# zprodev/zlib.es

Hardware: AMD Instinct MI355X
Metric: GiB/s deflate+inflate round trip, 64 MiB buffers (uncompressed bytes / wall), bit-exact vs reference (higher is better)
Workload: dtype u8; 1 GPU; random64: 1 x 64 MiB xorshift buffer(s) per GPU (seed 12345+index), deflate then inflate, HBM-resident; bytes_per_buffer=67108864, compressed_bytes=67176156, parallelism=independent buffers, one per GPU

## Files before the change

### zlib.es_amd/csrc/zes_api.hip

```cpp
#include "../../include/zes.h"
#include "zes_kernels.h"
#include "zes_chain.h"

#include <algorithm>
#include <atomic>
#include <condition_variable>
#include <cstdio>
#include <cstddef>
#include <cstdlib>
#include <cstring>
#include <chrono>
#include <functional>
#include <future>
#include <initializer_list>
#include <deque>
#include <map>
#include <mutex>
#include <string>
#include <thread>
#include <vector>

extern "C" int zes_gen(uint8_t* out, uint64_t n, uint32_t kind, uint32_t seed);

namespace {
// ... 808 lines not shown
  if ((rc = ensure(g.hists, (size_t)nblk * 320 * 4))) return rc;
  if ((rc = ensure(g.codes, (size_t)nblk * 320 * 4))) return rc;
  if ((rc = ensure(g.hdrs, (size_t)nblk * ZES_HDR_WORDS * 4))) return rc;
  if ((rc = ensure(g.adler, (size_t)nbuf * 16))) return rc;
  if ((rc = ensure(g.res, sizeof(ZesRes) * nbuf))) return rc;
  ZesBuf* dbufs = (ZesBuf*)g.bufs.p;
  ZesBlk* dblks = (ZesBlk*)g.blks.p;
  unsigned long long* adler = (unsigned long long*)g.adler.p;
  if (nbuf > 1) {
    if (nbuf <= DEFLATE_TABLE_BUFS) {
      memcpy(g.pinned->def.table, hb.data(), sizeof(ZesBuf) * nbuf);
      HIPCHK(hipMemcpyAsync(g.bufs.p, g.pinned->def.table, sizeof(ZesBuf) * nbuf, hipMemcpyHostToDevice, g.stream));
    } else {
      HIPCHK(hipMemcpy(g.bufs.p, hb.data(), sizeof(ZesBuf) * nbuf, hipMemcpyHostToDevice));
    }
  }
  {
    Timed t("k_make_blks");
    const uint32_t nthr = std::max(nblk, 2u * nbuf);
    hipLaunchKernelGGL(k_make_blks, dim3((nthr + 255) / 256), dim3(256), 0, g.stream, hb[0], nbuf, dbufs, dblks, nblk, adler);
  }
  {
    HIPCHK(hipEventRecord(g.ev_a0, g.stream));
    HIPCHK(hipStreamWaitEvent(g.s_adler, g.ev_a0, 0));
    Timed t("k_adler", g.s_adler);
    if (nbuf == 1) {
      const uint32_t nch = (uint32_t)((hb[0].n + ADLER_CHUNK - 1) / ADLER_CHUNK);
      hipLaunchKernelGGL(k_adler, dim3(nch), dim3(ADLER_THREADS), 0, g.s_adler, d_in, hb[0].in_off, hb[0].n, adler);
    } else {
      hipLaunchKernelGGL(k_adler_blocks, dim3(nblk), dim3(ADLER_THREADS), 0, g.s_adler, d_in, dbufs, dblks, adler);
    }
  }
  HIPCHK(hipEventRecord(g.ev_a1, g.s_adler));
  const bool sort_dbg = getenv("ZES_DEBUG_PHASES") != nullptr;
  if (sort_dbg && (rc = phases_arm(zes_sort_set_dbg, nblk))) return rc;
  static const bool use_index = getenv("ZES_NO_INDEX") == nullptr;
  rc = launch_lz77(d_in, nblk, use_index, nbuf > 1 && nblk > 256, sort_dbg, [&]() -> int {
    if (!sort_dbg) return ZES_OK;
    return phases_print(zes_sort_set_dbg, nblk, 7,
                        "zes sort steps (avg cycles over %u blocks): zero %.0f count %.0f flag %.0f compact %.0f stage %.0f three passes %.0f sd/inv %.0f\n");
  });
  if (rc) return rc;
  if (sort_dbg) {
    if ((rc = phases_print(zes_parse_set_dbg, nblk, 7, "zes parse steps (avg cycles over %u blocks): A %.0f B %.0f C %.0f D1 %.0f D2 %.0f D3 %.0f out %.0f\n"))) return rc;
    if ((rc = phases_arm(zes_huff_set_dbg, nblk))) return rc;
  }
  ZesRes* res_direct = (nbuf <= DEFLATE_DIRECT_BUFS && g.pinned_dev) ? g.pinned_dev->def.res : nullptr;
  {
    Timed t("k_huff");
    hipLaunchKernelGGL(k_huff, dim3(nblk), dim3(HUFF_THREADS_HOST), 0, g.stream, dblks, (const uint32_t*)g.hists.p,
                       (uint32_t*)g.codes.p, (uint32_t*)g.hdrs.p);
  }
  if (sort_dbg && (rc = phases_print(zes_huff_set_dbg, nblk, 7,
                                     "zes huff steps (avg cycles over %u blocks): lit/len lengths %.0f distance lengths %.0f codes %.0f run-length coding %.0f its code %.0f header bits %.0f totals+out %.0f\n")))
    return rc;
  {
    HIPCHK(hipStreamWaitEvent(g.stream, g.ev_a1, 0));
    Timed t("k_layout");
    hipLaunchKernelGGL(k_layout, dim3(nbuf), dim3(256), 0, g.stream, d_out, dbufs, dblks, adler, res_direct ? res_direct : (ZesRes*)g.res.p);
  }
  {
    Timed t("k_emit");
    hipLaunchKernelGGL(k_emit, dim3(nblk), dim3(EMIT_THREADS), 0, g.stream, d_out, dbufs, dblks, (uint32_t*)g.idx_a.p,
                       (const uint32_t*)g.codes.p, (const uint32_t*)g.hdrs.p);
  }
  HIPCHK(hipGetLastError());
  ZesRes* r = g.pinned->def.res;
  if (nbuf > DEFLATE_DIRECT_BUFS) {
    if (nbuf > g.res_more_n) {
      if (g.res_more) HIPCHK(hipHostFree(g.res_more));
      g.res_more = nullptr;
      g.res_more_n = 0;
      HIPCHK(hipHostMalloc((void**)&g.res_more, sizeof(ZesRes) * nbuf * 2, hipHostMallocDefault));
      g.res_more_n = (size_t)nbuf * 2;
    }
    r = g.res_more;
  }
  if (!res_direct) HIPCHK(hipMemcpyAsync(r, g.res.p, sizeof(ZesRes) * nbuf, hipMemcpyDeviceToHost, g.stream));
  if (one && one->defer) return ZES_OK;
  HIPCHK(hipStreamSynchronize(g.stream));
  collect_times();
  for (uint32_t k = 0; k < nbuf; k++) {
    out_len[live[k]] = r[k].out_len;
    status[live[k]] = r[k].status;
  }
  if (one) one->adler = r[0].aux;
  return ZES_OK;
}

int deflate_one(const uint8_t* d_in, uint64_t in_off, uint64_t n, uint8_t* d_out, uint64_t out_off, uint64_t cap, uint64_t* out_len,
                DeflateRange* range = nullptr) {
  int32_t st = 0;
  const int rc = deflate_batch_core(d_in, &in_off, &n, d_out, &out_off, &cap, out_len, &st, 1, range);
  return rc ? rc : st;
}

int read_res(ZesRes* out) {
  HIPCHK(hipMemcpyAsync(&g.pinned->res1, g.res.p, sizeof(ZesRes), hipMemcpyDeviceToHost, g.stream));
  HIPCHK(hipStreamSynchronize(g.stream));
  *out = g.pinned->res1;
  return ZES_OK;
}

struct InfJob {
  uint64_t in_off, c, out_off, cap;
  uint64_t out_len;
  int status;
// ... 4809 lines not shown
```

### zlib.es_amd/csrc/zes_deflate.hip

```cpp
#include "zes_common.h"
#include "zes_kernels.h"

__device__ static inline uint32_t lds_ld32u(const uint8_t* s, uint32_t off) {
  const uint32_t* w = reinterpret_cast<const uint32_t*>(s);
  uint32_t i = off >> 2;
  uint32_t lo = w[i], hi = w[i + 1];
  return __builtin_amdgcn_alignbyte(hi, lo, off & 3u);
}

__device__ static inline void stage_block(uint8_t* s, const uint8_t* g, uint32_t bytes, uint32_t padded) {
  const uint32_t tid = threadIdx.x, nth = blockDim.x;
  const uint32_t mis = (uint32_t)((uintptr_t)g & 15u);
  if (mis == 0) {
    const uint4* g4 = reinterpret_cast<const uint4*>(g);
    uint4* s4 = reinterpret_cast<uint4*>(s);
    const uint32_t full = bytes >> 4;
    for (uint32_t i = tid; i < full; i += nth) s4[i] = g4[i];
    for (uint32_t i = (full << 4) + tid; i < padded; i += nth) s[i] = i < bytes ? g[i] : (uint8_t)0;
  } else {
    for (uint32_t i = tid; i < padded; i += nth) s[i] = i < bytes ? g[i] : (uint8_t)0;
  }
}

__device__ unsigned long long* g_sort_dbg = nullptr;
// ... 1783 lines not shown
      const uint32_t c = cb + k;
      const unsigned long long mk = mks[k];
      if ((mk >> lane) & 1ull) {
        const uint32_t m = ism[k] ? mw[k] : 0u;
        const uint32_t rank = (uint32_t)__popcll(mk & zes_lanemask_lt());
        uint32_t tv;
        if (m & ZES_TOK_MATCH) {
          tv = m;
          atomicAdd(&S.lh[257u + zes_len_code(zes_tok_len(m))], 1u);
          atomicAdd(&S.dh[zes_dist_code(zes_tok_dist(m))], 1u);
        } else {
          tv = by[k];
          atomicAdd(&S.lh[tv], 1u);
        }
        to[S.u.d.cpre[c] + rank] = tv;
      }
    }
  }
  __syncthreads();
  PSTAMP(6);
  if (tid == 0) {
    S.lh[256] = 1;
    blks[g].ntok = total;
  }
  __syncthreads();
  uint32_t* hg = hists + (uint64_t)g * 320;
  for (uint32_t i = tid; i < 288; i += PARSE_THREADS) hg[i] = S.lh[i];
  if (tid < 32) hg[288 + tid] = S.dh[tid];
  PSTAMP(7);
}

__global__ __launch_bounds__(PARSE_THREADS) void k_lz_parse(const uint8_t* __restrict__ d_in, const ZesBuf* __restrict__ bufs,
                                                            ZesBlk* __restrict__ blks, const uint32_t* __restrict__ match_in,
                                                            uint32_t* __restrict__ tok_out, uint32_t* __restrict__ hists,
                                                            const uint32_t* __restrict__ tmask_all, const uint32_t* __restrict__ mlist_all) {
  __shared__ __align__(16) ParseSmemT<false> S;
  parse_body<false>(S, d_in, bufs, blks, match_in, tok_out, hists, tmask_all, mlist_all);
}
__global__ __launch_bounds__(PARSE_THREADS, 8) void k_lz_parse_small(const uint8_t* __restrict__ d_in, const ZesBuf* __restrict__ bufs,
                                                                     ZesBlk* __restrict__ blks, const uint32_t* __restrict__ match_in,
                                                                     uint32_t* __restrict__ tok_out, uint32_t* __restrict__ hists,
                                                                     const uint32_t* __restrict__ tmask_all,
                                                                     const uint32_t* __restrict__ mlist_all) {
  __shared__ __align__(16) ParseSmemT<true> S;
  parse_body<true>(S, d_in, bufs, blks, match_in, tok_out, hists, tmask_all, mlist_all);
}

__device__ unsigned long long* g_huff_dbg = nullptr;
void zes_huff_set_dbg(unsigned long long* p) { (void)hipMemcpyToSymbol(HIP_SYMBOL(g_huff_dbg), &p, sizeof p); }
#define USTAMP(i)                                                                                        \
  do {                                                                                                   \
    if (g_huff_dbg && threadIdx.x == 0) g_huff_dbg[(size_t)blockIdx.x * 8 + (i)] = (unsigned long long)clock64(); \
  } while (0)
#define HUFF_THREADS 256
#define PM_MAXN 288
struct HuffSmem {
  uint32_t hist[320];
  uint32_t lw[PM_MAXN];
  uint16_t lsym[PM_MAXN];
  uint32_t w[2][2 * PM_MAXN];
  uint32_t pk[PM_MAXN];
  uint16_t leafpos[15][PM_MAXN];
  uint32_t a_k[16];
  uint8_t lens[320];
  uint8_t clens[32];
  uint16_t codes[320];
  uint16_t ccodes[32];
  uint8_t rl_sym[320];
  uint8_t rl_val[320];
  uint32_t nrl;
  uint32_t hdr[ZES_HDR_WORDS];
  uint32_t hdr_bits;
  uint32_t total_bits;
  uint32_t ccount[16], cfirst[16], crun[16];
  uint16_t cwave[HUFF_THREADS / 64][16];
  uint8_t cl[320];
  uint16_t run_tok[320];
  uint32_t wsum[HUFF_THREADS / 64];
  unsigned long long starts[5];
};

__device__ static inline uint32_t lower_bound_u32(const uint32_t* a, uint32_t n, uint32_t v) {
  uint32_t lo = 0, hi = n;
  while (lo < hi) {
    uint32_t mid = (lo + hi) >> 1;
    if (a[mid] < v) lo = mid + 1; else hi = mid;
  }
  return lo;
}
__device__ static inline uint32_t upper_bound_u32(const uint32_t* a, uint32_t n, uint32_t v) {
  uint32_t lo = 0, hi = n;
  while (lo < hi) {
    uint32_t mid = (lo + hi) >> 1;
    if (a[mid] <= v) lo = mid + 1; else hi = mid;
  }
  return lo;
}

__device__ static void pm_lengths(HuffSmem& S, const uint32_t* hist, uint32_t nsym, uint32_t L, uint8_t* lens) {
  const uint32_t tid = threadIdx.x, lane = tid & 63u;
  __syncthreads();
  uint32_t n = 0;
  for (uint32_t s0 = 0; s0 < nsym; s0 += HUFF_THREADS) n += (uint32_t)__syncthreads_count(s0 + tid < nsym && hist[s0 + tid] != 0u);
  for (uint32_t s = tid; s < nsym; s += HUFF_THREADS) {
    lens[s] = 0;
    const uint32_t c = hist[s];
    if (c) {
      uint32_t rank = 0;
      for (uint32_t j = 0; j < nsym; j++) {
        const uint32_t cj = hist[j];
        rank += (cj != 0) && (cj < c || (cj == c && j < s));
      }
      S.lw[rank] = c;
      S.lsym[rank] = (uint16_t)s;
    }
  }
  __syncthreads();
  if (n == 0) return;
  if (n == 1) {
    if (tid == 0) lens[S.lsym[0]] = 1;
    __syncthreads();
    return;
  }
  for (uint32_t i = tid; i < n; i += HUFF_THREADS) {
    S.w[0][i] = S.lw[i];
    S.leafpos[0][i] = (uint16_t)i;
  }
  uint32_t len_prev = n & ~1u;
  uint32_t sel = 0;
  __syncthreads();
  static_assert(PM_MAXN <= 2 * HUFF_THREADS && PM_MAXN < 512, "two items of either kind per thread, nine search steps");
  const uint32_t st0 = 1u << (31u - (uint32_t)__builtin_clz(n));
  const bool wide = n > HUFF_THREADS;
  for (uint32_t k = 1; k < L; k++) {
    const uint32_t np = len_prev >> 1;
    const uint2* wp2 = reinterpret_cast<const uint2*>(S.w[sel]);
    uint32_t* wc = S.w[sel ^ 1];
    const uint32_t i0 = min(tid, n - 1u), i1 = min(tid + HUFF_THREADS, n - 1u);
    const uint32_t j0 = min(tid, np - 1u), j1 = min(tid + HUFF_THREADS, np - 1u);
    const uint32_t lv0 = S.lw[i0], lv1 = S.lw[i1];
    const uint2 pa = wp2[j0], pb = wp2[j1];
    const uint32_t pv0 = pa.x + pa.y, pv1 = pb.x + pb.y;
    uint32_t ll0 = 0, ll1 = 0, pl0 = 0, pl1 = 0;
    if (!wide) {
#pragma unroll 1
      for (uint32_t st = st0; st; st >>= 1) {
        const uint32_t ml = ll0 + st, mp = pl0 + st;
        const uint2 x = wp2[min(ml, np) - 1u];
        const uint32_t y = S.lw[min(mp, n) - 1u];
        ll0 = (ml <= np && x.x + x.y < lv0) ? ml : ll0;
        pl0 = (mp <= n && y <= pv0) ? mp : pl0;
      }
    } else {
#pragma unroll 1
      for (uint32_t st = st0; st; st >>= 1) {
        const uint32_t ml0 = ll0 + st, ml1 = ll1 + st, mp0 = pl0 + st, mp1 = pl1 + st;
        const uint2 x0 = wp2[min(ml0, np) - 1u], x1 = wp2[min(ml1, np) - 1u];
        const uint32_t y0 = S.lw[min(mp0, n) - 1u], y1 = S.lw[min(mp1, n) - 1u];
        ll0 = (ml0 <= np && x0.x + x0.y < lv0) ? ml0 : ll0;
        ll1 = (ml1 <= np && x1.x + x1.y < lv1) ? ml1 : ll1;
        pl0 = (mp0 <= n && y0 <= pv0) ? mp0 : pl0;
        pl1 = (mp1 <= n && y1 <= pv1) ? mp1 : pl1;
      }
    }
    if (tid < n) {
      wc[tid + ll0] = lv0;
      S.leafpos[k][tid] = (uint16_t)(tid + ll0);
    }
    if (tid < np) wc[tid + pl0] = pv0;
    if (wide) {
      if (tid + HUFF_THREADS < n) {
        wc[tid + HUFF_THREADS + ll1] = lv1;
        S.leafpos[k][tid + HUFF_THREADS] = (uint16_t)(tid + HUFF_THREADS + ll1);
      }
      if (tid + HUFF_THREADS < np) wc[tid + HUFF_THREADS + pl1] = pv1;
    }
    len_prev = (n + np) & ~1u;
    sel ^= 1;
    __syncthreads();
  }
  if (tid < 64u) {
    uint32_t m = len_prev;
    for (int k = (int)L - 1; k >= 0; k--) {
      uint32_t a = 0;
#pragma unroll
      for (uint32_t c = 0; c < (PM_MAXN + 63) / 64; c++) {
        const uint32_t i = c * 64u + lane;
        a += (uint32_t)__popcll(__ballot(i < n && S.leafpos[k][min(i, n - 1u)] < m));
      }
      if (lane == 0) S.a_k[k] = a;
      m = 2u * (m - a);
    }
  }
  __syncthreads();
  for (uint32_t i = tid; i < n; i += HUFF_THREADS) {
    uint32_t l = 0;
    for (uint32_t k = 0; k < L; k++) l += (S.a_k[k] > i);
    lens[S.lsym[i]] = (uint8_t)l;
  }
  __syncthreads();
}

__device__ static void canon_codes(HuffSmem& S, const uint8_t* lens, uint32_t nsym, uint16_t* codes) {
  const uint32_t tid = threadIdx.x, lane = tid & 63u, wave = tid >> 6;
  if (tid < 16) {
    S.ccount[tid] = 0;
    S.crun[tid] = 0;
  }
  __syncthreads();
  for (uint32_t s = tid; s < nsym; s += HUFF_THREADS)
    if (lens[s]) atomicAdd(&S.ccount[lens[s]], 1u);
  __syncthreads();
  if (tid == 0) {
    uint32_t code = 0;
    for (uint32_t l = 1; l < 16; l++) {
      S.cfirst[l] = code;
      code = (code + S.ccount[l]) << 1;
    }
  }
  for (uint32_t s0 = 0; s0 < nsym; s0 += HUFF_THREADS) {
    const uint32_t s = s0 + tid;
    const uint32_t l = s < nsym ? lens[s] : 0u;
    uint64_t same = ~0ull;
#pragma unroll
    for (int bt = 0; bt < 4; bt++) {
      const bool bit = (l >> bt) & 1u;
      const uint64_t bal = __ballot(bit);
      same &= bit ? bal : ~bal;
    }
    const uint32_t below = (uint32_t)__popcll(same & zes_lanemask_lt());
    if (lane < 16) S.cwave[wave][lane] = 0;
    __syncthreads();
    if (l && below == 0) S.cwave[wave][l] = (uint16_t)__popcll(same);
    __syncthreads();
    uint32_t code = 0;
    if (l) {
      uint32_t rank = S.crun[l] + below;
      for (uint32_t w = 0; w < wave; w++) rank += S.cwave[w][l];
      code = __brev(S.cfirst[l] + rank) >> (32u - l);
    }
    if (s < nsym) codes[s] = (uint16_t)code;
    __syncthreads();
    if (tid < 16) {
      uint32_t add = 0;
      for (uint32_t w = 0; w < HUFF_THREADS / 64; w++) add += S.cwave[w][tid];
      S.crun[tid] += add;
    }
  }
  __syncthreads();
}

__device__ static inline void hdr_or(HuffSmem& S, uint32_t bitpos, uint32_t value, uint32_t nbits) {
  const uint32_t w = bitpos >> 5, sh = bitpos & 31u;
  atomicOr(&S.hdr[w], value << sh);
  if (sh + nbits > 32u) atomicOr(&S.hdr[w + 1], value >> (32u - sh));
}

__global__ __launch_bounds__(HUFF_THREADS) void k_huff(ZesBlk* __restrict__ blks, const uint32_t* __restrict__ hists,
                                                       uint32_t* __restrict__ codes_out, uint32_t* __restrict__ hdr_out) {
  __shared__ HuffSmem S;
  const uint32_t g = blockIdx.x, tid = threadIdx.x;
  const uint32_t* hg = hists + (uint64_t)g * 320;
  for (uint32_t i = tid; i < 320; i += HUFF_THREADS) S.hist[i] = hg[i];
  for (uint32_t i = tid; i < ZES_HDR_WORDS; i += HUFF_THREADS) S.hdr[i] = 0;
  if (tid == 0) S.total_bits = 0;
  __syncthreads();

  USTAMP(0);
  pm_lengths(S, S.hist, 286, 15, S.lens);
  USTAMP(1);
  pm_lengths(S, S.hist + 288, 30, 15, S.lens + 288);
  USTAMP(2);
  canon_codes(S, S.lens, 286, S.codes);
  canon_codes(S, S.lens + 288, 30, S.codes + 288);
  USTAMP(3);

  const uint32_t lane = tid & 63u, wave = tid >> 6;
  if (tid == 0) {
    S.a_k[0] = 256;
    S.a_k[1] = 0;
    S.nrl = 0;
  }
  __syncthreads();
  if (tid < 29 && S.hist[257 + tid]) atomicMax(&S.a_k[0], 257u + tid);
  if (tid < 30 && S.hist[288 + tid]) atomicMax(&S.a_k[1], tid);
  __syncthreads();
  const uint32_t HLIT = S.a_k[0] + 1u, HDIST = S.a_k[1] + 1u, ncl = HLIT + HDIST;
  for (uint32_t i = tid; i < ncl; i += HUFF_THREADS) S.cl[i] = i < HLIT ? S.lens[i] : S.lens[288 + i - HLIT];
  if (tid < 32) S.hist[tid] = 0;
  __syncthreads();
#pragma unroll
  for (int q = 0; q < 2; q++) {
    const uint32_t i = tid + q * HUFF_THREADS;
    const bool st = i < 320u && (i >= ncl || i == 0 || S.cl[i] != S.cl[i - 1]);
    const uint64_t m = __ballot(st);
    if (lane == 0 && (i >> 6) < 5u) S.starts[i >> 6] = m;
  }
  __syncthreads();
  uint32_t mytok[2] = {0, 0}, myn[2] = {0, 0};
#pragma unroll
  for (int q = 0; q < 2; q++) {
    const uint32_t i = tid + q * HUFF_THREADS;
    if (i < ncl && (i == 0 || S.cl[i] != S.cl[i - 1])) {
      const uint32_t v = S.cl[i];
      uint32_t nxt = ncl;
      {
        uint32_t wd = (i + 1u) >> 6;
        uint64_t mm = wd < 5u ? (S.starts[wd] & (~0ull << ((i + 1u) & 63u))) : 0ull;
        while (wd < 5u && mm == 0ull) {
          wd++;
          mm = wd < 5u ? S.starts[wd] : 0ull;
        }
        if (wd < 5u) nxt = min(ncl, wd * 64u + (uint32_t)__builtin_ctzll(mm));
      }
      const uint32_t n = nxt - i;
      const uint32_t cap = v ? 6u : 138u, per = v ? 2u : 1u;
      const uint32_t m = n % cap;
      myn[q] = n;
      mytok[q] = (n / cap) * per + (m >= 4u ? per : m);
    }
  }
  uint32_t pre[2];
#pragma unroll
  for (int q = 0; q < 2; q++) {
    uint32_t incl = mytok[q];
#pragma unroll
    for (int d = 1; d < 64; d <<= 1) {
      const uint32_t t = __shfl_up(incl, d);
      if ((int)lane >= d) incl += t;
    }
    if (lane == 63) S.wsum[wave] = incl;
    __syncthreads();
    uint32_t base = S.nrl;
    for (uint32_t w = 0; w < wave; w++) base += S.wsum[w];
    pre[q] = base + incl - mytok[q];
    __syncthreads();
    if (tid == HUFF_THREADS - 1) S.nrl = pre[q] + mytok[q];
    __syncthreads();
  }
#pragma unroll
  for (int q = 0; q < 2; q++) {
    if (myn[q]) {
      const uint32_t v = S.cl[tid + q * HUFF_THREADS];
      const uint32_t cap = v ? 6u : 138u;
      uint32_t pos = pre[q], rem = myn[q];
      while (rem) {
        const uint32_t r = min(rem, cap);
        if (r >= 4u) {
          if (v == 0) {
            S.rl_sym[pos] = (r >= 11u) ? 18 : 17;
            S.rl_val[pos] = (uint8_t)r;
            pos++;
          } else {
            S.rl_sym[pos] = (uint8_t)v;
            S.rl_val[pos] = 1;
            pos++;
            S.rl_sym[pos] = 16;
            S.rl_val[pos] = (uint8_t)(r - 1u);
            pos++;
          }
        } else {
          for (uint32_t j = 0; j < r; j++) {
            S.rl_sym[pos] = (uint8_t)v;
            S.rl_val[pos] = 1;
            pos++;
          }
        }
        rem -= r;
      }
    }
  }
  __syncthreads();
  const uint32_t nrl = S.nrl;
  for (uint32_t i = tid; i < nrl; i += HUFF_THREADS) atomicAdd(&S.hist[S.rl_sym[i]], 1u);
  __syncthreads();
  USTAMP(4);
  pm_lengths(S, S.hist, 19, 7, S.clens);
  canon_codes(S, S.clens, 19, S.ccodes);
  USTAMP(5);

  if (tid == 0) S.a_k[2] = 4;
  __syncthreads();
  if (tid < 19 && S.clens[kClOrder[tid]]) atomicMax(&S.a_k[2], tid + 1u);
  __syncthreads();
  const uint32_t HCLEN = S.a_k[2];
  if (tid == 0) atomicOr(&S.hdr[0], (HLIT - 257u) | ((HDIST - 1u) << 5) | (((HCLEN - 4u) & 15u) << 10));
  if (tid < HCLEN) {
    uint32_t bp = 14u + 3u * tid;
    hdr_or(S, bp, S.clens[kClOrder[tid]], 3);
  }
  uint32_t tv[2] = {0, 0}, tb[2] = {0, 0};
#pragma unroll
  for (int q = 0; q < 2; q++) {
    const uint32_t i = 2u * tid + (uint32_t)q;
    if (i < nrl) {
      const uint32_t sy = S.rl_sym[i], cl = S.clens[sy];
      const uint32_t xb = sy == 18u ? 7u : sy == 17u ? 3u : sy == 16u ? 2u : 0u;
      const uint32_t xv = sy == 18u ? S.rl_val[i] - 11u : (sy == 17u || sy == 16u) ? S.rl_val[i] - 3u : 0u;
      tv[q] = (uint32_t)S.ccodes[sy] | (xv << cl);
      tb[q] = cl + xb;
    }
  }
  {
    const uint32_t mine = tb[0] + tb[1];
    uint32_t incl = mine;
#pragma unroll
    for (int d = 1; d < 64; d <<= 1) {
      const uint32_t t = __shfl_up(incl, d);
      if ((int)lane >= d) incl += t;
    }
    if (lane == 63) S.wsum[wave] = incl;
    __syncthreads();
    uint32_t base = 14u + 3u * HCLEN, total = 0;
    for (uint32_t w = 0; w < HUFF_THREADS / 64; w++) {
      if (w < wave) base += S.wsum[w];
      total += S.wsum[w];
    }
    uint32_t bp = base + incl - mine;
    if (tb[0]) hdr_or(S, bp, tv[0], tb[0]);
    bp += tb[0];
    if (tb[1]) hdr_or(S, bp, tv[1], tb[1]);
    if (tid == 0) S.hdr_bits = 14u + 3u * HCLEN + total;
  }
  __syncthreads();
  USTAMP(6);
  uint32_t part = 0;
  for (uint32_t s = tid; s < 286; s += HUFF_THREADS) {
    uint32_t xb = (s >= 257) ? kLenXbits[s - 257] : 0u;
    part += hg[s] * ((uint32_t)S.lens[s] + xb);
  }
  if (tid < 30) part += hg[288 + tid] * ((uint32_t)S.lens[288 + tid] + kDistXbits[tid]);
  atomicAdd(&S.total_bits, part);
  __syncthreads();
  if (tid == 0) {
    blks[g].hdr_bits = S.hdr_bits;
    blks[g].bits = 3u + S.hdr_bits + S.total_bits;
  }
  uint32_t* cg = codes_out + (uint64_t)g * 320;
  for (uint32_t i = tid; i < 320; i += HUFF_THREADS) cg[i] = (uint32_t)S.codes[i] | ((uint32_t)S.lens[i] << 16);
  uint32_t* hd = hdr_out + (uint64_t)g * ZES_HDR_WORDS;
  for (uint32_t i = tid; i < ZES_HDR_WORDS; i += HUFF_THREADS) hd[i] = S.hdr[i];
  USTAMP(7);
}

__global__ __launch_bounds__(HUFF_THREADS) void k_huff_lengths_only(const uint32_t* __restrict__ hist, uint32_t nsym, uint32_t L,
                                                                    uint8_t* __restrict__ lens_out) {
  __shared__ HuffSmem S;
  const uint32_t tid = threadIdx.x;
  for (uint32_t i = tid; i < 320; i += HUFF_THREADS) S.hist[i] = i < nsym ? hist[i] : 0u;
  __syncthreads();
  pm_lengths(S, S.hist, nsym, L, S.lens);
  for (uint32_t i = tid; i < nsym; i += HUFF_THREADS) lens_out[i] = S.lens[i];
}

__global__ void k_make_blks(ZesBuf b0, uint32_t nbuf, ZesBuf* __restrict__ bufs, ZesBlk* __restrict__ blks, uint32_t nblk,
                            unsigned long long* __restrict__ adler) {
  const uint32_t i = blockIdx.x * blockDim.x + threadIdx.x;
  if (nbuf == 1u && i == 0) bufs[0] = b0;
  if (i < 2u * nbuf) adler[i] = 0ull;
  if (i >= nblk) return;
  uint32_t lo = 0, hi = nbuf;
  while (hi - lo > 1) {
    const uint32_t mid = (lo + hi) >> 1;
    if ((nbuf == 1u ? b0.first_blk : bufs[mid].first_blk) <= i) lo = mid; else hi = mid;
  }
  const uint64_t n = nbuf == 1u ? b0.n : bufs[lo].n;
  const uint32_t fb = nbuf == 1u ? b0.first_blk : bufs[lo].first_blk;
  ZesBlk z;
  z.buf = lo;
  z.blk = i - fb;
  z.len = (uint32_t)min((uint64_t)ZES_BLK, n - (uint64_t)z.blk * ZES_BLK);
  z.ntok = 0;
  z.hdr_bits = 0;
  z.bits = 0;
  z.bit_off = 0;
  blks[i] = z;
}

__device__ __forceinline__ static void adler_group_sums(uint4 v, uint32_t& a, uint32_t& w) {
  a = __builtin_amdgcn_udot4(v.x, 0x01010101u, 0u, false);
  a = __builtin_amdgcn_udot4(v.y, 0x01010101u, a, false);
  a = __builtin_amdgcn_udot4(v.z, 0x01010101u, a, false);
  a = __builtin_amdgcn_udot4(v.w, 0x01010101u, a, false);
  w = __builtin_amdgcn_udot4(v.x, 0x0D0E0F10u, 0u, false);
  w = __builtin_amdgcn_udot4(v.y, 0x090A0B0Cu, w, false);
  w = __builtin_amdgcn_udot4(v.z, 0x05060708u, w, false);
  w = __builtin_amdgcn_udot4(v.w, 0x01020304u, w, false);
}

__device__ __forceinline__ static void adler_chunk(const uint8_t* __restrict__ p0, uint64_t n, uint64_t c0, uint64_t clen,
                                                   unsigned long long* __restrict__ acc) {
  __shared__ uint64_t sa[ADLER_THREADS / 64], sb[ADLER_THREADS / 64];
  const uint32_t tid = threadIdx.x, lane = tid & 63u, wave = tid >> 6;
  const uint8_t* p = p0 + c0;
  uint64_t A = 0, B = 0;
  const bool aligned = (((uintptr_t)p) & 15u) == 0;
  uint64_t o_first = (uint64_t)tid * 16;
  if (aligned) {
    constexpr uint64_t ROUND = (uint64_t)ADLER_THREADS * 16 * 4;
    const uint64_t nround = clen / ROUND;
    for (uint64_t r = 0; r < nround; r++) {
      uint4 v[4];
#pragma unroll
      for (uint32_t q = 0; q < 4; q++) v[q] = *reinterpret_cast<const uint4*>(p + r * ROUND + (uint64_t)q * ADLER_THREADS * 16 + (uint64_t)tid * 16);
#pragma unroll
// ... 445 lines not shown
```

### zlib.es_amd/csrc/zes_kernels.h

```cpp
#pragma once
#include "zes_common.h"

#define SORT_THREADS 1024
#define SORT_WAVES (SORT_THREADS / 64)
#ifndef MATCH_THREADS
#define MATCH_THREADS 1024
#endif
#define IDX_THREADS 1024
#define ZES_SORT_LAZY 0x80000000u
#define ZES_SORT_INDEX 0x40000000u
#define ZES_SORT_REDO 0x20000000u
#define ZES_INV_NONE 0xFFFFFFFFu
#define ZES_ROUTE_WORDS 9u
#define ZES_ROUTE_SORT_TWO 1u
#define ZES_ROUTE_SORT_DENSE 2u
#define ZES_ROUTE_IDX_MAXC 0x3FFFFu
#define ZES_ROUTE_IDX_GROUP 0x40000000u
#define ZES_ROUTE_IDX_HEAVY 0x80000000u
#define ZES_ROUTE_GUARDED 1u
#define ZES_ROUTE_PROBED 2u
#define ZES_ROUTE_PERIODIC 4u
#define ZES_ROUTE_ABORT3 8u
#define ZES_ROUTE_LATE_CLEAR 16u
#define ZES_ROUTE_WALK3 32u
#define PARSE_THREADS 1024
#define EMIT_THREADS 1024
#define HUFF_THREADS_HOST 256
#define ADLER_THREADS 256
#define ADLER_CHUNK 65536u
#define CRC_THREADS 256u
#define CRC_PIECES 16u
#define CRC_CHUNK (CRC_THREADS * CRC_PIECES * 16u)
#define CRC_STRIDE (CRC_THREADS * 16u)
#define CRC_TAB_FOLD 512u
#define CRC_TAB_LANE 640u
#define CRC_TAB_POW (CRC_TAB_LANE + CRC_THREADS)
#define ZES_PAR_DBG_ROW 32
#define ZES_TMASK_WORDS (131072 / 32 + 4)
#define ZES_MLIST_CAP 4095u
#define ZES_MLIST_WORDS 4096u
#define PAR_THREADS 1024
#define PAR_WAVES (PAR_THREADS / 64)
#define INF_SCAN_THREADS 256
#ifndef INF_SCAN_BYTES
#define INF_SCAN_BYTES 8192u
#endif
#define SEG_BUCKETS 2048u

struct ZesInfBuf {
  uint64_t in_off, c, out_off, cap;
  uint32_t first_chunk;
  uint32_t cand_base;
  uint32_t cand_cap;
  uint32_t work_first;
  uint32_t start_rel;
  uint32_t own_rel;
  uint32_t range_flags;
  uint32_t pad;
};
#define ZES_START_ANY 1u
#define ZES_OWN_ONLY 2u

#define ZES_WORK_AUTO 0xFFFFFFFFu

struct ZesCandRes {
  uint64_t end_bit;
  uint32_t out_len;
  uint32_t flags;
};

struct ZesParMirror {
  ZesCandRes* cres_host;
  uint32_t* start_host;
  const uint32_t* counters;
  uint32_t* counters_host;
  uint32_t counter_words;
};

struct ZesSegRes {
  uint64_t end_bit;
// ... 253 lines not shown
```

Baseline: 45.88 GiB/s.

## Build lit/len and distance Huffman trees concurrently in one 384-thread block

The Huffman kernel grows to 384 threads and splits into a 320-thread lit/len team and a 64-thread distance wavefront, so both package-merge length computations and canonical code assignments run at the same time instead of back to back. The rank sort now reads keys as uint4 vectors. The code-length alphabet runs on a single wavefront using waitcnt instead of block barriers, and the per-thread loops collapse to one item per thread. This is meant to cut serial latency in k_huff, which runs once per block. In exchange the block is larger, uses more LDS, and leans on wave-level synchronisation that assumes 64-wide waves.

```diff
diff --git a/zlib.es_amd/csrc/zes_api.hip b/zlib.es_amd/csrc/zes_api.hip
--- a/zlib.es_amd/csrc/zes_api.hip
+++ b/zlib.es_amd/csrc/zes_api.hip
@@ -884,7 +884,7 @@
                        (uint32_t*)g.codes.p, (uint32_t*)g.hdrs.p);
   }
   if (sort_dbg && (rc = phases_print(zes_huff_set_dbg, nblk, 7,
-                                     "zes huff steps (avg cycles over %u blocks): lit/len lengths %.0f distance lengths %.0f codes %.0f run-length coding %.0f its code %.0f header bits %.0f totals+out %.0f\n")))
+                                     "zes huff steps (avg cycles over %u blocks): rank sorts %.0f both alphabets' levels %.0f codes %.0f run-length coding %.0f its code %.0f header bits %.0f totals+out %.0f\n")))
     return rc;
   {
     HIPCHK(hipStreamWaitEvent(g.stream, g.ev_a1, 0));
diff --git a/zlib.es_amd/csrc/zes_deflate.hip b/zlib.es_amd/csrc/zes_deflate.hip
--- a/zlib.es_amd/csrc/zes_deflate.hip
+++ b/zlib.es_amd/csrc/zes_deflate.hip
@@ -1859,202 +1859,178 @@
   do {                                                                                                   \
     if (g_huff_dbg && threadIdx.x == 0) g_huff_dbg[(size_t)blockIdx.x * 8 + (i)] = (unsigned long long)clock64(); \
   } while (0)
-#define HUFF_THREADS 256
-#define PM_MAXN 288
+#define HUFF_THREADS 384
+#define HUFF_WAVES (HUFF_THREADS / 64)
+#define PM_MAXN 320
+static_assert(HUFF_THREADS == HUFF_THREADS_HOST && HUFF_THREADS == PM_MAXN + 64, "the lit/len team and the distance wavefront");
 struct HuffSmem {
   uint32_t hist[320];
-  uint32_t lw[PM_MAXN];
-  uint16_t lsym[PM_MAXN];
-  uint32_t w[2][2 * PM_MAXN];
-  uint32_t pk[PM_MAXN];
-  uint16_t leafpos[15][PM_MAXN];
-  uint32_t a_k[16];
+  alignas(16) uint32_t key[320];
+  uint32_t lw[320];
+  uint16_t lsym[320];
+  alignas(8) uint32_t w[2][640];
+  uint16_t leafpos[15][320];
+  uint32_t pm_n[2];
+  uint32_t a_k[2][16];
+  uint32_t top[3];
   uint8_t lens[320];
   uint8_t clens[32];
   uint16_t codes[320];
   uint16_t ccodes[32];
   uint8_t rl_sym[320];
   uint8_t rl_val[320];
-  uint32_t nrl;
   uint32_t hdr[ZES_HDR_WORDS];
   uint32_t hdr_bits;
   uint32_t total_bits;
-  uint32_t ccount[16], cfirst[16], crun[16];
-  uint16_t cwave[HUFF_THREADS / 64][16];
+  uint32_t ccount[2][16], cfirst[2][16];
+  uint16_t cwave[HUFF_WAVES][16];
   uint8_t cl[320];
-  uint16_t run_tok[320];
-  uint32_t wsum[HUFF_THREADS / 64];
+  uint32_t wsum[HUFF_WAVES];
   unsigned long long starts[5];
 };
 
-__device__ static inline uint32_t lower_bound_u32(const uint32_t* a, uint32_t n, uint32_t v) {
-  uint32_t lo = 0, hi = n;
-  while (lo < hi) {
-    uint32_t mid = (lo + hi) >> 1;
-    if (a[mid] < v) lo = mid + 1; else hi = mid;
-  }
-  return lo;
-}
-__device__ static inline uint32_t upper_bound_u32(const uint32_t* a, uint32_t n, uint32_t v) {
-  uint32_t lo = 0, hi = n;
-  while (lo < hi) {
-    uint32_t mid = (lo + hi) >> 1;
-    if (a[mid] <= v) lo = mid + 1; else hi = mid;
-  }
-  return lo;
-}
-
-__device__ static void pm_lengths(HuffSmem& S, const uint32_t* hist, uint32_t nsym, uint32_t L, uint8_t* lens) {
-  const uint32_t tid = threadIdx.x, lane = tid & 63u;
-  __syncthreads();
-  uint32_t n = 0;
-  for (uint32_t s0 = 0; s0 < nsym; s0 += HUFF_THREADS) n += (uint32_t)__syncthreads_count(s0 + tid < nsym && hist[s0 + tid] != 0u);
-  for (uint32_t s = tid; s < nsym; s += HUFF_THREADS) {
-    lens[s] = 0;
-    const uint32_t c = hist[s];
-    if (c) {
-      uint32_t rank = 0;
-      for (uint32_t j = 0; j < nsym; j++) {
-        const uint32_t cj = hist[j];
-        rank += (cj != 0) && (cj < c || (cj == c && j < s));
-      }
-      S.lw[rank] = c;
-      S.lsym[rank] = (uint16_t)s;
-    }
-  }
-  __syncthreads();
-  if (n == 0) return;
-  if (n == 1) {
-    if (tid == 0) lens[S.lsym[0]] = 1;
-    __syncthreads();
-    return;
-  }
-  for (uint32_t i = tid; i < n; i += HUFF_THREADS) {
-    S.w[0][i] = S.lw[i];
-    S.leafpos[0][i] = (uint16_t)i;
-  }
+struct PmTeam {
+  uint32_t t, size, base;
+};
+template <bool kWave>
+__device__ __forceinline__ static void pm_sync() {
+  if (kWave) asm volatile("s_waitcnt lgkmcnt(0)" ::: "memory");
+  else __syncthreads();
+}
+
+template <bool kWave>
+__device__ static void pm_lengths(HuffSmem& S, const PmTeam T, uint32_t nsym, uint32_t L, uint8_t* lens, int stamp) {
+  const uint32_t lane = threadIdx.x & 63u, b = T.base, a = b ? 1u : 0u;
+  const uint32_t i = T.t < T.size ? T.t : PM_MAXN;
+  const uint32_t key = (i < nsym ? S.hist[b + i] : 0u) - 1u;
+  if (i < (b ? 32u : 288u)) S.key[b + i] = key;
+  if (T.t == 0) S.pm_n[a] = 0;
+  if (i < nsym) lens[i] = 0;
+  pm_sync<kWave>();
+  const bool used = key != ~0u;
+  uint32_t rank = 0;
+  if (used) {
+    const uint32_t own = __builtin_amdgcn_readfirstlane(i & ~63u);
+    const uint4* k4 = reinterpret_cast<const uint4*>(S.key + b);
+    for (uint32_t q = 0; q < own >> 2; q++) {
+      const uint4 k = k4[q];
+      rank += (k.x <= key) + (k.y <= key) + (k.z <= key) + (k.w <= key);
+    }
+    for (uint32_t q = own >> 2, qe = min(own + 64u, (nsym + 3u) & ~3u) >> 2; q < qe; q++) {
+      const uint4 k = k4[q];
+      const uint32_t j = 4u * q;
+      rank += (k.x < key || (k.x == key && j < i)) + (k.y < key || (k.y == key && j + 1u < i)) +
+              (k.z < key || (k.z == key && j + 2u < i)) + (k.w < key || (k.w == key && j + 3u < i));
+    }
+    for (uint32_t q = (own + 64u) >> 2, qe = (nsym + 3u) >> 2; q < qe; q++) {
+      const uint4 k = k4[q];
+      rank += (k.x < key) + (k.y < key) + (k.z < key) + (k.w < key);
+    }
+    S.lw[b + rank] = key + 1u;
+    S.lsym[b + rank] = (uint16_t)i;
+    S.w[0][2u * b + rank] = key + 1u;
+    S.leafpos[0][b + rank] = (uint16_t)rank;
+  }
+  {
+    const uint32_t cnt = (uint32_t)__popcll(__ballot(used));
+    if (lane == 0 && cnt) atomicAdd(&S.pm_n[a], cnt);
+  }
+  pm_sync<kWave>();
+  const uint32_t n = S.pm_n[a];
+  if (stamp >= 0) USTAMP(stamp);
+  if (n == 1 && T.t == 0) lens[S.lsym[b]] = 1;
+  const bool merge = n >= 2u;
+  const bool mine = merge && i < n;
+  const uint32_t lv = mine ? S.lw[b + i] : 0u;
   uint32_t len_prev = n & ~1u;
   uint32_t sel = 0;
-  __syncthreads();
-  static_assert(PM_MAXN <= 2 * HUFF_THREADS && PM_MAXN < 512, "two items of either kind per thread, nine search steps");
-  const uint32_t st0 = 1u << (31u - (uint32_t)__builtin_clz(n));
-  const bool wide = n > HUFF_THREADS;
+  const uint32_t st0 = merge ? 1u << (31u - (uint32_t)__builtin_clz(n)) : 0u;
   for (uint32_t k = 1; k < L; k++) {
     const uint32_t np = len_prev >> 1;
-    const uint2* wp2 = reinterpret_cast<const uint2*>(S.w[sel]);
-    uint32_t* wc = S.w[sel ^ 1];
-    const uint32_t i0 = min(tid, n - 1u), i1 = min(tid + HUFF_THREADS, n - 1u);
-    const uint32_t j0 = min(tid, np - 1u), j1 = min(tid + HUFF_THREADS, np - 1u);
-    const uint32_t lv0 = S.lw[i0], lv1 = S.lw[i1];
-    const uint2 pa = wp2[j0], pb = wp2[j1];
-    const uint32_t pv0 = pa.x + pa.y, pv1 = pb.x + pb.y;
-    uint32_t ll0 = 0, ll1 = 0, pl0 = 0, pl1 = 0;
-    if (!wide) {
+    const uint2* wp2 = reinterpret_cast<const uint2*>(S.w[sel] + 2u * b);
+    uint32_t* wc = S.w[sel ^ 1] + 2u * b;
+    if (mine) {
+      const uint2 pa = wp2[min(i, np - 1u)];
+      const uint32_t pv = pa.x + pa.y;
+      uint32_t ll = 0, pl = 0;
 #pragma unroll 1
       for (uint32_t st = st0; st; st >>= 1) {
-        const uint32_t ml = ll0 + st, mp = pl0 + st;
+        const uint32_t ml = ll + st, mp = pl + st;
         const uint2 x = wp2[min(ml, np) - 1u];
-        const uint32_t y = S.lw[min(mp, n) - 1u];
-        ll0 = (ml <= np && x.x + x.y < lv0) ? ml : ll0;
-        pl0 = (mp <= n && y <= pv0) ? mp : pl0;
-      }
-    } else {
-#pragma unroll 1
-      for (uint32_t st = st0; st; st >>= 1) {
-        const uint32_t ml0 = ll0 + st, ml1 = ll1 + st, mp0 = pl0 + st, mp1 = pl1 + st;
-        const uint2 x0 = wp2[min(ml0, np) - 1u], x1 = wp2[min(ml1, np) - 1u];
-        const uint32_t y0 = S.lw[min(mp0, n) - 1u], y1 = S.lw[min(mp1, n) - 1u];
-        ll0 = (ml0 <= np && x0.x + x0.y < lv0) ? ml0 : ll0;
-        ll1 = (ml1 <= np && x1.x + x1.y < lv1) ? ml1 : ll1;
-        pl0 = (mp0 <= n && y0 <= pv0) ? mp0 : pl0;
-        pl1 = (mp1 <= n && y1 <= pv1) ? mp1 : pl1;
-      }
-    }
-    if (tid < n) {
-      wc[tid + ll0] = lv0;
-      S.leafpos[k][tid] = (uint16_t)(tid + ll0);
-    }
-    if (tid < np) wc[tid + pl0] = pv0;
-    if (wide) {
-      if (tid + HUFF_THREADS < n) {
-        wc[tid + HUFF_THREADS + ll1] = lv1;
-        S.leafpos[k][tid + HUFF_THREADS] = (uint16_t)(tid + HUFF_THREADS + ll1);
-      }
-      if (tid + HUFF_THREADS < np) wc[tid + HUFF_THREADS + pl1] = pv1;
+        const uint32_t y = S.lw[b + min(mp, n) - 1u];
+        ll = (ml <= np && x.x + x.y < lv) ? ml : ll;
+        pl = (mp <= n && y <= pv) ? mp : pl;
+      }
+      wc[i + ll] = lv;
+      S.leafpos[k][b + i] = (uint16_t)(i + ll);
+      if (i < np) wc[i + pl] = pv;
     }
     len_prev = (n + np) & ~1u;
     sel ^= 1;
-    __syncthreads();
-  }
-  if (tid < 64u) {
+    pm_sync<kWave>();
+  }
+  if (merge && T.t < 64u) {
     uint32_t m = len_prev;
     for (int k = (int)L - 1; k >= 0; k--) {
-      uint32_t a = 0;
-#pragma unroll
-      for (uint32_t c = 0; c < (PM_MAXN + 63) / 64; c++) {
-        const uint32_t i = c * 64u + lane;
-        a += (uint32_t)__popcll(__ballot(i < n && S.leafpos[k][min(i, n - 1u)] < m));
-      }
-      if (lane == 0) S.a_k[k] = a;
-      m = 2u * (m - a);
-    }
-  }
-  __syncthreads();
-  for (uint32_t i = tid; i < n; i += HUFF_THREADS) {
+      uint32_t cnt = 0;
+#pragma unroll
+      for (uint32_t c0 = 0; c0 < PM_MAXN; c0 += 64u) {
+        const uint32_t j = c0 + lane;
+        cnt += (uint32_t)__popcll(__ballot(j < n && S.leafpos[k][b + min(j, n - 1u)] < m));
+      }
+      if (lane == 0) S.a_k[a][k] = cnt;
+      m = 2u * (m - cnt);
+    }
+  }
+  pm_sync<kWave>();
+  if (mine) {
     uint32_t l = 0;
-    for (uint32_t k = 0; k < L; k++) l += (S.a_k[k] > i);
-    lens[S.lsym[i]] = (uint8_t)l;
-  }
-  __syncthreads();
-}
-
-__device__ static void canon_codes(HuffSmem& S, const uint8_t* lens, uint32_t nsym, uint16_t* codes) {
-  const uint32_t tid = threadIdx.x, lane = tid & 63u, wave = tid >> 6;
-  if (tid < 16) {
-    S.ccount[tid] = 0;
-    S.crun[tid] = 0;
-  }
-  __syncthreads();
-  for (uint32_t s = tid; s < nsym; s += HUFF_THREADS)
-    if (lens[s]) atomicAdd(&S.ccount[lens[s]], 1u);
-  __syncthreads();
-  if (tid == 0) {
+    for (uint32_t k = 0; k < L; k++) l += (S.a_k[a][k] > i);
+    lens[S.lsym[b + i]] = (uint8_t)l;
+  }
+  pm_sync<kWave>();
+}
+
+template <bool kWave>
+__device__ static void canon_codes(HuffSmem& S, const PmTeam T, const uint8_t* lens, uint32_t nsym, uint16_t* codes) {
+  const uint32_t lane = threadIdx.x & 63u, wave = threadIdx.x >> 6, a = T.base ? 1u : 0u;
+  const uint32_t wave0 = wave - (T.t >> 6);
+  const bool sym = T.t < T.size && T.t < nsym;
+  if (T.t < 16) S.ccount[a][T.t] = 0;
+  if (lane < 16) S.cwave[wave][lane] = 0;
+  pm_sync<kWave>();
+  const uint32_t l = sym ? lens[T.t] : 0u;
+  uint64_t same = ~0ull;
+#pragma unroll
+  for (int bt = 0; bt < 4; bt++) {
+    const bool bit = (l >> bt) & 1u;
+    const uint64_t bal = __ballot(bit);
+    same &= bit ? bal : ~bal;
+  }
+  const uint32_t below = (uint32_t)__popcll(same & zes_lanemask_lt());
+  if (l && below == 0) {
+    S.cwave[wave][l] = (uint16_t)__popcll(same);
+    atomicAdd(&S.ccount[a][l], (uint32_t)__popcll(same));
+  }
+  pm_sync<kWave>();
+  if (T.t == 0) {
     uint32_t code = 0;
-    for (uint32_t l = 1; l < 16; l++) {
-      S.cfirst[l] = code;
-      code = (code + S.ccount[l]) << 1;
-    }
-  }
-  for (uint32_t s0 = 0; s0 < nsym; s0 += HUFF_THREADS) {
-    const uint32_t s = s0 + tid;
-    const uint32_t l = s < nsym ? lens[s] : 0u;
-    uint64_t same = ~0ull;
-#pragma unroll
-    for (int bt = 0; bt < 4; bt++) {
-      const bool bit = (l >> bt) & 1u;
-      const uint64_t bal = __ballot(bit);
-      same &= bit ? bal : ~bal;
-    }
-    const uint32_t below = (uint32_t)__popcll(same & zes_lanemask_lt());
-    if (lane < 16) S.cwave[wave][lane] = 0;
-    __syncthreads();
-    if (l && below == 0) S.cwave[wave][l] = (uint16_t)__popcll(same);
-    __syncthreads();
+    for (uint32_t k = 1; k < 16; k++) {
+      S.cfirst[a][k] = code;
+      code = (code + S.ccount[a][k]) << 1;
+    }
+  }
+  pm_sync<kWave>();
+  if (sym) {
     uint32_t code = 0;
     if (l) {
-      uint32_t rank = S.crun[l] + below;
-      for (uint32_t w = 0; w < wave; w++) rank += S.cwave[w][l];
-      code = __brev(S.cfirst[l] + rank) >> (32u - l);
-    }
-    if (s < nsym) codes[s] = (uint16_t)code;
-    __syncthreads();
-    if (tid < 16) {
-      uint32_t add = 0;
-      for (uint32_t w = 0; w < HUFF_THREADS / 64; w++) add += S.cwave[w][tid];
-      S.crun[tid] += add;
-    }
-  }
-  __syncthreads();
+      uint32_t rank = below;
+      for (uint32_t w = wave0; w < wave; w++) rank += S.cwave[w][l];
+      code = __brev(S.cfirst[a][l] + rank) >> (32u - l);
+    }
+    codes[T.t] = (uint16_t)code;
+  }
+  pm_sync<kWave>();
 }
 
 __device__ static inline void hdr_or(HuffSmem& S, uint32_t bitpos, uint32_t value, uint32_t nbits) {
@@ -2067,47 +2043,49 @@
                                                        uint32_t* __restrict__ codes_out, uint32_t* __restrict__ hdr_out) {
   __shared__ HuffSmem S;
   const uint32_t g = blockIdx.x, tid = threadIdx.x;
+  const uint32_t lane = tid & 63u, wave = __builtin_amdgcn_readfirstlane(tid >> 6);
   const uint32_t* hg = hists + (uint64_t)g * 320;
-  for (uint32_t i = tid; i < 320; i += HUFF_THREADS) S.hist[i] = hg[i];
+  if (tid < 320) {
+    S.hist[tid] = hg[tid];
+    S.lens[tid] = 0;
+    S.codes[tid] = 0;
+  }
   for (uint32_t i = tid; i < ZES_HDR_WORDS; i += HUFF_THREADS) S.hdr[i] = 0;
   if (tid == 0) S.total_bits = 0;
   __syncthreads();
 
   USTAMP(0);
-  pm_lengths(S, S.hist, 286, 15, S.lens);
-  USTAMP(1);
-  pm_lengths(S, S.hist + 288, 30, 15, S.lens + 288);
-  USTAMP(2);
-  canon_codes(S, S.lens, 286, S.codes);
-  canon_codes(S, S.lens + 288, 30, S.codes + 288);
+  {
+    const bool ll = wave < PM_MAXN / 64u;
+    const PmTeam T = ll ? PmTeam{tid, PM_MAXN, 0u} : PmTeam{lane, 64u, 288u};
+    const uint32_t nsym = ll ? 286u : 30u;
+    pm_lengths<false>(S, T, nsym, 15, S.lens + T.base, 1);
+    USTAMP(2);
+    canon_codes<false>(S, T, S.lens + T.base, nsym, S.codes + T.base);
+  }
   USTAMP(3);
 
-  const uint32_t lane = tid & 63u, wave = tid >> 6;
   if (tid == 0) {
-    S.a_k[0] = 256;
-    S.a_k[1] = 0;
-    S.nrl = 0;
-  }
-  __syncthreads();
-  if (tid < 29 && S.hist[257 + tid]) atomicMax(&S.a_k[0], 257u + tid);
-  if (tid < 30 && S.hist[288 + tid]) atomicMax(&S.a_k[1], tid);
-  __syncthreads();
-  const uint32_t HLIT = S.a_k[0] + 1u, HDIST = S.a_k[1] + 1u, ncl = HLIT + HDIST;
-  for (uint32_t i = tid; i < ncl; i += HUFF_THREADS) S.cl[i] = i < HLIT ? S.lens[i] : S.lens[288 + i - HLIT];
+    S.top[0] = 256;
+    S.top[1] = 0;
+  }
+  __syncthreads();
+  if (tid < 29 && S.hist[257 + tid]) atomicMax(&S.top[0], 257u + tid);
+  if (tid < 30 && S.hist[288 + tid]) atomicMax(&S.top[1], tid);
+  __syncthreads();
+  const uint32_t HLIT = S.top[0] + 1u, HDIST = S.top[1] + 1u, ncl = HLIT + HDIST;
+  if (tid < ncl) S.cl[tid] = tid < HLIT ? S.lens[tid] : S.lens[288 + tid - HLIT];
   if (tid < 32) S.hist[tid] = 0;
   __syncthreads();
-#pragma unroll
-  for (int q = 0; q < 2; q++) {
-    const uint32_t i = tid + q * HUFF_THREADS;
-    const bool st = i < 320u && (i >= ncl || i == 0 || S.cl[i] != S.cl[i - 1]);
+  {
+    const bool st = tid < 320u && (tid >= ncl || tid == 0 || S.cl[tid] != S.cl[tid - 1]);
     const uint64_t m = __ballot(st);
-    if (lane == 0 && (i >> 6) < 5u) S.starts[i >> 6] = m;
-  }
-  __syncthreads();
-  uint32_t mytok[2] = {0, 0}, myn[2] = {0, 0};
-#pragma unroll
-  for (int q = 0; q < 2; q++) {
-    const uint32_t i = tid + q * HUFF_THREADS;
+    if (lane == 0 && wave < 5u) S.starts[wave] = m;
+  }
+  __syncthreads();
+  uint32_t mytok = 0, myn = 0;
+  {
+    const uint32_t i = tid;
     if (i < ncl && (i == 0 || S.cl[i] != S.cl[i - 1])) {
       const uint32_t v = S.cl[i];
       uint32_t nxt = ncl;
@@ -2123,14 +2101,13 @@
       const uint32_t n = nxt - i;
       const uint32_t cap = v ? 6u : 138u, per = v ? 2u : 1u;
       const uint32_t m = n % cap;
-      myn[q] = n;
-      mytok[q] = (n / cap) * per + (m >= 4u ? per : m);
-    }
-  }
-  uint32_t pre[2];
-#pragma unroll
-  for (int q = 0; q < 2; q++) {
-    uint32_t incl = mytok[q];
+      myn = n;
+      mytok = (n / cap) * per + (m >= 4u ? per : m);
+    }
+  }
+  uint32_t pre, nrl = 0;
+  {
+    uint32_t incl = mytok;
 #pragma unroll
     for (int d = 1; d < 64; d <<= 1) {
       const uint32_t t = __shfl_up(incl, d);
@@ -2138,19 +2115,18 @@
     }
     if (lane == 63) S.wsum[wave] = incl;
     __syncthreads();
-    uint32_t base = S.nrl;
-    for (uint32_t w = 0; w < wave; w++) base += S.wsum[w];
-    pre[q] = base + incl - mytok[q];
-    __syncthreads();
-    if (tid == HUFF_THREADS - 1) S.nrl = pre[q] + mytok[q];
-    __syncthreads();
-  }
-#pragma unroll
-  for (int q = 0; q < 2; q++) {
-    if (myn[q]) {
-      const uint32_t v = S.cl[tid + q * HUFF_THREADS];
+    uint32_t base = 0;
+    for (uint32_t w = 0; w < 5u; w++) {
+      if (w < wave) base += S.wsum[w];
+      nrl += S.wsum[w];
+    }
+    pre = base + incl - mytok;
+  }
+  {
+    if (myn) {
+      const uint32_t v = S.cl[tid];
       const uint32_t cap = v ? 6u : 138u;
-      uint32_t pos = pre[q], rem = myn[q];
+      uint32_t pos = pre, rem = myn;
       while (rem) {
         const uint32_t r = min(rem, cap);
         if (r >= 4u) {
@@ -2178,39 +2154,35 @@
     }
   }
   __syncthreads();
-  const uint32_t nrl = S.nrl;
-  for (uint32_t i = tid; i < nrl; i += HUFF_THREADS) atomicAdd(&S.hist[S.rl_sym[i]], 1u);
+  if (tid < nrl) atomicAdd(&S.hist[S.rl_sym[tid]], 1u);
   __syncthreads();
   USTAMP(4);
-  pm_lengths(S, S.hist, 19, 7, S.clens);
-  canon_codes(S, S.clens, 19, S.ccodes);
+  if (wave == 0) {
+    const PmTeam T{lane, 64u, 0u};
+    pm_lengths<true>(S, T, 19, 7, S.clens, -1);
+    canon_codes<true>(S, T, S.clens, 19, S.ccodes);
+    const uint64_t used = __ballot(lane < 19 && S.clens[kClOrder[min(lane, 18u)]]);
+    if (lane == 0) S.top[2] = max(4u, 64u - (uint32_t)__builtin_clzll(used | 1ull));
+  }
+  __syncthreads();
   USTAMP(5);
 
-  if (tid == 0) S.a_k[2] = 4;
-  __syncthreads();
-  if (tid < 19 && S.clens[kClOrder[tid]]) atomicMax(&S.a_k[2], tid + 1u);
-  __syncthreads();
-  const uint32_t HCLEN = S.a_k[2];
+  const uint32_t HCLEN = S.top[2];
   if (tid == 0) atomicOr(&S.hdr[0], (HLIT - 257u) | ((HDIST - 1u) << 5) | (((HCLEN - 4u) & 15u) << 10));
   if (tid < HCLEN) {
     uint32_t bp = 14u + 3u * tid;
     hdr_or(S, bp, S.clens[kClOrder[tid]], 3);
   }
-  uint32_t tv[2] = {0, 0}, tb[2] = {0, 0};
-#pragma unroll
-  for (int q = 0; q < 2; q++) {
-    const uint32_t i = 2u * tid + (uint32_t)q;
-    if (i < nrl) {
-      const uint32_t sy = S.rl_sym[i], cl = S.clens[sy];
-      const uint32_t xb = sy == 18u ? 7u : sy == 17u ? 3u : sy == 16u ? 2u : 0u;
-      const uint32_t xv = sy == 18u ? S.rl_val[i] - 11u : (sy == 17u || sy == 16u) ? S.rl_val[i] - 3u : 0u;
-      tv[q] = (uint32_t)S.ccodes[sy] | (xv << cl);
-      tb[q] = cl + xb;
-    }
+  uint32_t tv = 0, tb = 0;
+  if (tid < nrl) {
+    const uint32_t sy = S.rl_sym[tid], cl = S.clens[sy];
+    const uint32_t xb = sy == 18u ? 7u : sy == 17u ? 3u : sy == 16u ? 2u : 0u;
+    const uint32_t xv = sy == 18u ? S.rl_val[tid] - 11u : (sy == 17u || sy == 16u) ? S.rl_val[tid] - 3u : 0u;
+    tv = (uint32_t)S.ccodes[sy] | (xv << cl);
+    tb = cl + xb;
   }
   {
-    const uint32_t mine = tb[0] + tb[1];
-    uint32_t incl = mine;
+    uint32_t incl = tb;
 #pragma unroll
     for (int d = 1; d < 64; d <<= 1) {
       const uint32_t t = __shfl_up(incl, d);
@@ -2219,32 +2191,26 @@
     if (lane == 63) S.wsum[wave] = incl;
     __syncthreads();
     uint32_t base = 14u + 3u * HCLEN, total = 0;
-    for (uint32_t w = 0; w < HUFF_THREADS / 64; w++) {
+    for (uint32_t w = 0; w < 5u; w++) {
       if (w < wave) base += S.wsum[w];
       total += S.wsum[w];
     }
-    uint32_t bp = base + incl - mine;
-    if (tb[0]) hdr_or(S, bp, tv[0], tb[0]);
-    bp += tb[0];
-    if (tb[1]) hdr_or(S, bp, tv[1], tb[1]);
+    if (tb) hdr_or(S, base + incl - tb, tv, tb);
     if (tid == 0) S.hdr_bits = 14u + 3u * HCLEN + total;
   }
   __syncthreads();
   USTAMP(6);
   uint32_t part = 0;
-  for (uint32_t s = tid; s < 286; s += HUFF_THREADS) {
-    uint32_t xb = (s >= 257) ? kLenXbits[s - 257] : 0u;
-    part += hg[s] * ((uint32_t)S.lens[s] + xb);
-  }
+  if (tid < 286) part = hg[tid] * ((uint32_t)S.lens[tid] + (tid >= 257 ? kLenXbits[tid - 257] : 0u));
   if (tid < 30) part += hg[288 + tid] * ((uint32_t)S.lens[288 + tid] + kDistXbits[tid]);
-  atomicAdd(&S.total_bits, part);
+  if (tid < 320) atomicAdd(&S.total_bits, part);
   __syncthreads();
   if (tid == 0) {
     blks[g].hdr_bits = S.hdr_bits;
     blks[g].bits = 3u + S.hdr_bits + S.total_bits;
   }
   uint32_t* cg = codes_out + (uint64_t)g * 320;
-  for (uint32_t i = tid; i < 320; i += HUFF_THREADS) cg[i] = (uint32_t)S.codes[i] | ((uint32_t)S.lens[i] << 16);
+  if (tid < 320) cg[tid] = (uint32_t)S.codes[tid] | ((uint32_t)S.lens[tid] << 16);
   uint32_t* hd = hdr_out + (uint64_t)g * ZES_HDR_WORDS;
   for (uint32_t i = tid; i < ZES_HDR_WORDS; i += HUFF_THREADS) hd[i] = S.hdr[i];
   USTAMP(7);
@@ -2253,11 +2219,13 @@
 __global__ __launch_bounds__(HUFF_THREADS) void k_huff_lengths_only(const uint32_t* __restrict__ hist, uint32_t nsym, uint32_t L,
                                                                     uint8_t* __restrict__ lens_out) {
   __shared__ HuffSmem S;
-  const uint32_t tid = threadIdx.x;
-  for (uint32_t i = tid; i < 320; i += HUFF_THREADS) S.hist[i] = i < nsym ? hist[i] : 0u;
-  __syncthreads();
-  pm_lengths(S, S.hist, nsym, L, S.lens);
-  for (uint32_t i = tid; i < nsym; i += HUFF_THREADS) lens_out[i] = S.lens[i];
+  const uint32_t tid = threadIdx.x, wave = __builtin_amdgcn_readfirstlane(tid >> 6);
+  if (tid < 320) S.hist[tid] = tid < nsym ? hist[tid] : 0u;
+  __syncthreads();
+  if (nsym > 64u) pm_lengths<false>(S, PmTeam{tid, PM_MAXN, 0u}, nsym, L, S.lens, -1);
+  else if (wave == 0) pm_lengths<true>(S, PmTeam{tid, 64u, 0u}, nsym, L, S.lens, -1);
+  __syncthreads();
+  if (tid < nsym) lens_out[tid] = S.lens[tid];
 }
 
 __global__ void k_make_blks(ZesBuf b0, uint32_t nbuf, ZesBuf* __restrict__ bufs, ZesBlk* __restrict__ blks, uint32_t nblk,
diff --git a/zlib.es_amd/csrc/zes_kernels.h b/zlib.es_amd/csrc/zes_kernels.h
--- a/zlib.es_amd/csrc/zes_kernels.h
+++ b/zlib.es_amd/csrc/zes_kernels.h
@@ -25,7 +25,7 @@
 #define ZES_ROUTE_WALK3 32u
 #define PARSE_THREADS 1024
 #define EMIT_THREADS 1024
-#define HUFF_THREADS_HOST 256
+#define HUFF_THREADS_HOST 384
 #define ADLER_THREADS 256
 #define ADLER_CHUNK 65536u
 #define CRC_THREADS 256u
```

Result: faster. 47.06 GiB/s, median of 6 (+2.6%).
